# Piletskii-Oleg/chunkfs

Hardware: AMD Instinct MI355X
Metric: GiB/s chunked device-resident, FastCDC 4/8/16 KiB avg, at 1/2/4/8 MI355X (higher is better)
Workload: dtype u8

## Files before the change

chunkfs_amd/csrc/fastcdc.hip:

```cpp
#include "fastcdc.hpp"

#include <cstdlib>
#include <type_traits>

namespace cdc {
namespace p3 {
namespace {


constexpr uint32_t kCandPosMask = 0x00FFFFFFu;
constexpr uint32_t kCandHitL = 1u << 30;
constexpr uint32_t kCandHitS = 1u << 31;

typedef unsigned int u32x4 __attribute__((ext_vector_type(4)));
typedef const __attribute__((address_space(1))) u32x4 g_u32x4;
typedef const __attribute__((address_space(1))) uint8_t g_u8;
typedef const __attribute__((address_space(1))) uint32_t g_u32;
typedef __attribute__((address_space(1))) uint64_t g_u64;
__device__ __forceinline__ g_u32x4 *as_global4(const void *p) { return (g_u32x4 *)(p); }
__device__ __forceinline__ g_u8 *as_global1(const void *p) { return (g_u8 *)(p); }
__device__ __forceinline__ uint4 ld16(g_u32x4 *p) {
    const u32x4 v = *p;
    return make_uint4(v.x, v.y, v.z, v.w);
}
__device__ __forceinline__ uint4 ld16_nt(g_u32x4 *p) {
    const u32x4 v = __builtin_nontemporal_load(p);
    return make_uint4(v.x, v.y, v.z, v.w);
}

#ifndef CDC_SCAN_NOFENCE
#define SCHED_FENCE() __builtin_amdgcn_sched_barrier(0)
#else
#define SCHED_FENCE() do {} while (0)
#endif
#ifndef CDC_SCAN_WAVES
#define CDC_SCAN_WAVES 12
#endif
#ifndef CDC_SCAN_NT_ODD
#define CDC_SCAN_NT_ODD 1
#endif
#ifndef CDC_SCAN_WAVE_MAJOR
#define CDC_SCAN_WAVE_MAJOR 1
#endif
#ifndef CDC_SCAN_LOOK
#define CDC_SCAN_LOOK 1
#endif
#ifndef CDC_SCAN_TRUNC
#define CDC_SCAN_TRUNC 0
#endif

__device__ __forceinline__ void wave_sync_lds() {
    __builtin_amdgcn_fence(__ATOMIC_RELEASE, "wavefront");
    __builtin_amdgcn_wave_barrier();
    __builtin_amdgcn_fence(__ATOMIC_ACQUIRE, "wavefront");
}

__device__ __forceinline__ void locate(const StreamTable &st, uint64_t g, uint32_t &si, uint64_t &off) {
    uint32_t lo = 0, hi = st.n;
    while (hi - lo > 1) {
        const uint32_t mid = (lo + hi) >> 1;
        if (st.span_base[mid] <= g) lo = mid; else hi = mid;
    }
    si = lo;
    off = (g - st.span_base[lo]) << st.span_log2;
}

template <bool kAlign>
__device__ __forceinline__ uint32_t cand_test(uint64_t h, const FastParams &fp) {
    if constexpr (kAlign) {
        return (uint32_t)(h >> 32) & fp.cm32;
    } else {
        return ((uint32_t)h & fp.cm_lo) | ((uint32_t)(h >> 32) & fp.cm_hi);
    }
}

__device__ __forceinline__ uint64_t shl1_add(uint64_t h, uint64_t g) {
    return (h << 1) + g;
}

__device__ __forceinline__ uint64_t wave_shr1(uint64_t v, uint64_t fill) {
    const uint32_t lo = (uint32_t)__builtin_amdgcn_update_dpp(
        (int)(uint32_t)fill, (int)(uint32_t)v, 0x138, 0xF, 0xF, false);
    const uint32_t hi = (uint32_t)__builtin_amdgcn_update_dpp(
        (int)(uint32_t)(fill >> 32), (int)(uint32_t)(v >> 32), 0x138, 0xF, 0xF, false);
    return ((uint64_t)hi << 32) | lo;
}

__device__ __forceinline__ uint64_t readlane_u64(uint64_t v, int l) {
    const uint32_t lo = (uint32_t)__builtin_amdgcn_readlane((int)(uint32_t)v, l);
    const uint32_t hi = (uint32_t)__builtin_amdgcn_readlane((int)(uint32_t)(v >> 32), l);
    return ((uint64_t)hi << 32) | lo;
}

__device__ __forceinline__ uint64_t gear_prefix(uint64_t g, uint32_t lane) {
#pragma unroll
    for (int k = 1; k < 64; k <<= 1) {
        const uint64_t t = __shfl_up(g, k);
        if (lane >= (uint32_t)k) g += t << k;
    }
    return g;
}

constexpr uint32_t kTruncMax = 47;
constexpr uint32_t kTruncNone = 63;
constexpr uint32_t kTruncUnknown = 62;
constexpr int kRecTShift = 24;

struct Regime {
    uint64_t rem, a0, ce, re, tl;
};

__device__ __forceinline__ Regime regime(const FastParams &fp, uint64_t s, uint64_t n) {
    Regime R;
    uint64_t rem = n - s, center = fp.avg;
    if (rem > fp.max) rem = fp.max; else if (rem < center) center = rem;
    R.rem = rem;
    R.a0 = (fp.min / 2) * 2;
    R.ce = (center / 2) * 2;
    R.re = (rem / 2) * 2;
    R.tl = min(R.a0 + (uint64_t)fp.trunc, R.re);
    return R;
}


constexpr int kCopies = 32;
constexpr uint32_t kEntCap = 64;
constexpr uint32_t kStep = 64;

__device__ __forceinline__ uint64_t gear_of(const uint64_t *tab, uint32_t rep_off, uint32_t w, int b) {
    const uint32_t addr = __builtin_amdgcn_perm(rep_off, w, 0x0c0c0004u | ((uint32_t)b << 8));
    return *reinterpret_cast<const uint64_t *>(reinterpret_cast<const char *>(tab) + addr);
}

struct G4 {
    uint64_t v[4];
};

__device__ __forceinline__ void look4(G4 &g, const uint64_t *tab, uint32_t rep, uint32_t w) {
#pragma unroll
    for (int b = 0; b < 4; ++b) g.v[b] = gear_of(tab, rep, w, b);
}

template <bool kAlign>
__device__ __forceinline__ void chain4_test(uint64_t &h, uint32_t &acc, const G4 &g, const FastParams &fp) {
#pragma unroll
    for (int i = 0; i < 4; ++i) {
        h = shl1_add(h, g.v[i]);
        acc = min(acc, cand_test<kAlign>(h, fp));
    }
}

__device__ __forceinline__ uint32_t word_of(const uint4 &v, int w) {
    return w == 0 ? v.x : w == 1 ? v.y : w == 2 ? v.z : v.w;
}

__device__ __forceinline__ uint4 ld16_guarded(const uint8_t *base, uint32_t p, uint32_t limit) {
    if (p + 16 <= limit) return ld16(as_global4(base + p));
    uint32_t w[4] = {0, 0, 0, 0};
    if (p < limit) {
        g_u8 *gb = as_global1(base);
        for (uint32_t j = 0; p + j < limit; ++j) w[j >> 2] |= (uint32_t)gb[p + j] << (8 * j);
    }
    return make_uint4(w[0], w[1], w[2], w[3]);
}

struct EntryList {
    uint32_t *pos, *hlo, *hhi, *cnt;
};

constexpr uint32_t kEntFix = 1u << 31;
constexpr uint32_t kEntPos = kEntFix - 1;

__device__ __forceinline__ void append_hits(bool hit, uint32_t pos, uint64_t h0, uint32_t &ne,
                                            const EntryList &E) {
    const uint64_t m = __ballot(hit);
    if (m) {
        if (hit) {
            const uint32_t below = __builtin_amdgcn_mbcnt_hi((uint32_t)(m >> 32),
                                                             __builtin_amdgcn_mbcnt_lo((uint32_t)m, 0u));
            const uint32_t slot = ne + below;
            if (slot < kEntCap) {
                E.pos[slot] = pos;
                E.hlo[slot] = (uint32_t)h0;
                E.hhi[slot] = (uint32_t)(h0 >> 32);
            }
        }
        ne += (uint32_t)__popcll(m);
    }
}

__device__ __forceinline__ void append_hits_d(bool hit, uint32_t pos, uint64_t h0, const uint4 &q, uint32_t &ne,
                                              const EntryList &E, uint4 *edat) {
    const uint64_t m = __ballot(hit);
    if (m) {
        if (hit) {
            const uint32_t below = __builtin_amdgcn_mbcnt_hi((uint32_t)(m >> 32),
                                                             __builtin_amdgcn_mbcnt_lo((uint32_t)m, 0u));
            const uint32_t slot = ne + below;
            if (slot < kEntCap) {
                E.pos[slot] = pos;
                E.hlo[slot] = (uint32_t)h0;
                E.hhi[slot] = (uint32_t)(h0 >> 32);
                edat[slot] = q;
            }
        }
        ne += (uint32_t)__popcll(m);
    }
}

template <bool kAlign>
__device__ __forceinline__ uint32_t quarter(uint64_t &h, const uint4 &v, const uint64_t *tab, uint32_t rep,
                                            const FastParams &fp) {
    G4 ga, gb;
    uint32_t acc = 0xffffffffu;
    look4(ga, tab, rep, v.x);
    SCHED_FENCE();
    look4(gb, tab, rep, v.y);
    SCHED_FENCE();
    chain4_test<kAlign>(h, acc, ga, fp);
    SCHED_FENCE();
    look4(ga, tab, rep, v.z);
    SCHED_FENCE();
    chain4_test<kAlign>(h, acc, gb, fp);
    SCHED_FENCE();
    look4(gb, tab, rep, v.w);
    SCHED_FENCE();
    chain4_test<kAlign>(h, acc, ga, fp);
    SCHED_FENCE();
    chain4_test<kAlign>(h, acc, gb, fp);
    SCHED_FENCE();
    return acc;
}

struct Q4 {
    uint4 q[4];
};

template <bool kAlign, int kLook>
__device__ __forceinline__ void process_step(const Q4 &C, uint64_t &h, uint32_t pos0, uint32_t &ne,
                                             const EntryList &E, const uint64_t *tab, uint32_t rep,
                                             const FastParams &fp) {
    if constexpr (kLook == 1) {
        G4 ga, gb;
        look4(ga, tab, rep, C.q[0].x);
        SCHED_FENCE();
#pragma unroll
        for (int q = 0; q < 4; ++q) {
            const uint64_t h0 = h;
            uint32_t acc = 0xffffffffu;
#pragma unroll
            for (int w = 0; w < 4; w += 2) {
                look4(gb, tab, rep, word_of(C.q[q], w + 1));
                SCHED_FENCE();
                chain4_test<kAlign>(h, acc, ga, fp);
                SCHED_FENCE();
                if (q < 3 || w < 2) {
                    look4(ga, tab, rep, w < 2 ? word_of(C.q[q], w + 2) : word_of(C.q[q + 1], 0));
                    SCHED_FENCE();
                }
                chain4_test<kAlign>(h, acc, gb, fp);
                SCHED_FENCE();
            }
            append_hits(acc == 0, pos0 + 16 * q, h0, ne, E);
        }
    } else {
        G4 ga0, ga1, gb0, gb1;
        look4(ga0, tab, rep, C.q[0].x);
        look4(ga1, tab, rep, C.q[0].y);
        SCHED_FENCE();
#pragma unroll
        for (int q = 0; q < 4; ++q) {
            const uint64_t h0 = h;
            uint32_t acc = 0xffffffffu;
            look4(gb0, tab, rep, C.q[q].z);
            look4(gb1, tab, rep, C.q[q].w);
            SCHED_FENCE();
            chain4_test<kAlign>(h, acc, ga0, fp);
            chain4_test<kAlign>(h, acc, ga1, fp);
            SCHED_FENCE();
            if (q < 3) {
                look4(ga0, tab, rep, C.q[q + 1].x);
                look4(ga1, tab, rep, C.q[q + 1].y);
                SCHED_FENCE();
            }
            chain4_test<kAlign>(h, acc, gb0, fp);
            chain4_test<kAlign>(h, acc, gb1, fp);
            SCHED_FENCE();
            append_hits(acc == 0, pos0 + 16 * q, h0, ne, E);
        }
    }
}

template <bool kAlign>
__device__ __forceinline__ void process_step_d(const Q4 &C, uint64_t &h, uint32_t pos0, uint32_t &ne,
                                               const EntryList &E, uint4 *edat, const uint64_t *tab, uint32_t rep,
                                               const FastParams &fp) {
    G4 ga, gb;
    look4(ga, tab, rep, C.q[0].x);
    SCHED_FENCE();
#pragma unroll
    for (int q = 0; q < 4; ++q) {
        const uint64_t h0 = h;
        uint32_t acc = 0xffffffffu;
#pragma unroll
        for (int w = 0; w < 4; w += 2) {
            look4(gb, tab, rep, word_of(C.q[q], w + 1));
            SCHED_FENCE();
            chain4_test<kAlign>(h, acc, ga, fp);
            SCHED_FENCE();
            if (q < 3 || w < 2) {
                look4(ga, tab, rep, w < 2 ? word_of(C.q[q], w + 2) : word_of(C.q[q + 1], 0));
                SCHED_FENCE();
            }
            chain4_test<kAlign>(h, acc, gb, fp);
            SCHED_FENCE();
        }
        append_hits_d(acc == 0, pos0 + 16 * q, h0, C.q[q], ne, E, edat);
    }
}

template <bool kNt = false>
__device__ __forceinline__ void gload_step(Q4 &X, const uint8_t *gp, uint64_t istride, uint32_t t) {
#pragma unroll
    for (int i = 0; i < 4; ++i)
        X.q[i] = kNt ? ld16_nt(as_global4(gp + i * istride + t * kStep)) : ld16(as_global4(gp + i * istride + t * kStep));
}

__device__ __forceinline__ void stage_step(Q4 &C, const Q4 &X, uint4 *wrow, const uint4 *rrow) {
#pragma unroll
    for (int i = 0; i < 4; ++i) wrow[i * 16 * 5] = X.q[i];
    __builtin_amdgcn_wave_barrier();
#pragma unroll
    for (int k = 0; k < 4; ++k) C.q[k] = rrow[k];
    __builtin_amdgcn_wave_barrier();
}

typedef const __attribute__((address_space(3))) uint64_t lds_u64;
typedef const __attribute__((address_space(3))) char lds_char;

#if CDC_SCAN_TRUNC
__device__ __noinline__ uint32_t scan_trunc(const uint8_t *base, uint32_t c, uint64_t avail, lds_u64 *ltab,
                                            uint32_t rep, uint32_t mn, uint32_t avg, uint32_t mx, uint32_t trunc,
                                            uint64_t mask_s, uint64_t mask_l) {
    const uint32_t a0 = (mn / 2) * 2, ce = (avg / 2) * 2, re = (mx / 2) * 2;
    if (avail - c < (uint64_t)mx || (uint64_t)a0 + 52 > avail - c) return kTruncUnknown;
    const uint32_t tl = min(a0 + trunc, re);
    if (tl <= a0) return kTruncNone;
    const uint32_t len = tl - a0;
    const uint64_t w0 = (uint64_t)c + a0;
    const uint64_t al = w0 & ~3ull;
    const uint32_t sh = (uint32_t)(w0 - al);
    uint32_t w[13];
#pragma unroll
    for (int i = 0; i < 13; ++i) w[i] = *(g_u32 *)(base + al + 4 * i);
    uint64_t h = 0;
    uint32_t t = kTruncNone;
#pragma unroll
    for (int k = 0; k < 12; ++k) {
        const uint32_t a = __builtin_amdgcn_alignbyte(w[k + 1], w[k], sh);
#pragma unroll
        for (int j = 0; j < 4; ++j) {
            const uint32_t d = 4 * k + j;
            if (d >= kTruncMax) break;
            const uint32_t addr = __builtin_amdgcn_perm(rep, a, 0x0c0c0004u | ((uint32_t)j << 8));
            h = shl1_add(h, *reinterpret_cast<lds_u64 *>(reinterpret_cast<lds_char *>(ltab) + addr));
            const bool hit = d < len && !(h & ((a0 + d) < ce ? mask_s : mask_l));
            t = (hit && t == kTruncNone) ? d : t;
        }
    }
    return t;
}

#endif

__device__ __forceinline__ void flush_span(uint64_t g, const uint8_t *base, uint32_t span_len, uint64_t avail,
                                           uint32_t sub_mask, uint32_t ne, const EntryList &E, const uint64_t *tab,
                                           uint32_t rep, const FastParams &fp, const Candidates &cand,
                                           uint32_t lane, const uint4 *edat = nullptr) {
    wave_sync_lds();
    uint32_t *cpos = cand.pos + g * cand.cap;
    if (ne > kEntCap) {
        if (lane == 0) cand.count[g] = cand.cap + 1;
        wave_sync_lds();
        return;
    }
    uint32_t hs = 0, hl = 0, my_pos = 0;
    const uint32_t wd = lane < ne ? E.pos[lane] : 0u;
    const bool keep = lane < ne && ((wd & kEntFix) || (wd & sub_mask) >= 48);
    if (lane < ne) E.cnt[lane] = 0;
    if (keep) {
        my_pos = wd & kEntPos;
        uint64_t hh = ((uint64_t)E.hhi[lane] << 32) | E.hlo[lane];
        const uint4 v = edat ? edat[lane] : ld16_guarded(base, my_pos, span_len);
#pragma unroll
        for (int w = 0; w < 4; ++w)
#pragma unroll
            for (int b = 0; b < 4; ++b) {
                const int j = 4 * w + b;
                hh = (hh << 1) + gear_of(tab, rep, word_of(v, w), b);
                if (my_pos + j < span_len) {
                    hs |= (uint32_t)((hh & fp.mask_s_sh) == 0) << j;
                    hl |= (uint32_t)((hh & fp.mask_l_sh) == 0) << j;
                }
            }
        E.cnt[lane] = __popc(hs | hl);
    }
    wave_sync_lds();
    uint32_t slot = 0, total = 0;
    for (uint32_t k = 0; k < ne; ++k) {
        const uint32_t c = E.cnt[k];
        total += c;
        if ((E.pos[k] & kEntPos) < my_pos) slot += c;
    }
    if (keep) {
        for (uint32_t m = hs | hl; m; m &= m - 1) {
            const uint32_t j = __builtin_ctz(m);
            uint32_t t = kTruncUnknown;
#if CDC_SCAN_TRUNC
            t = scan_trunc(base, my_pos + j, avail, (lds_u64 *)tab, rep, fp.min, fp.avg, fp.max, fp.trunc,
                           fp.mask_s_sh, fp.mask_l_sh);
#endif
            if (slot < cand.cap)
                cpos[slot] = (my_pos + j) | (t << kRecTShift) | (((hs >> j) & 1u) << 31) | (((hl >> j) & 1u) << 30);
            ++slot;
        }
    }
    if (lane == 0) cand.count[g] = total;
    wave_sync_lds();
}

template <int kW>
struct ScanLds {
    uint64_t tab[256 * kCopies];
    uint4 stage[kW][64 * 5];
    uint32_t epos[kW][kEntCap];
    uint32_t ehlo[kW][kEntCap];
    uint32_t ehhi[kW][kEntCap];
    uint32_t ecnt[kW][kEntCap];
};

template <bool kAlign, int kW, int kLook, int kMode>
__global__ __launch_bounds__(kW * 64, 1) void scan_kernel(const StreamTable st, const FastParams fp,
                                                           const uint64_t *__restrict__ gear,
                                                           const Candidates cand, const Compact cp) {
    __shared__ ScanLds<kW> L;
    const uint64_t *tab = L.tab;
    for (int i = threadIdx.x; i < 256 * kCopies; i += kW * 64)
        L.tab[i] = gear[i / kCopies] << fp.tshift;
    if (blockIdx.x == 0 && threadIdx.x < kStatWords) cp.stats[threadIdx.x] = 0;
    __syncthreads();

    const uint32_t lane = threadIdx.x & 63;
    const uint32_t wave = threadIdx.x >> 6;
    const uint32_t rep = (lane & 31) * 8;
    const uint64_t span = 1ull << st.span_log2;
    const uint32_t sub_log2 = st.span_log2 - 6;
    const uint32_t sub = 1u << sub_log2;
    const uint32_t steps = sub / kStep;
    const uint32_t lo = lane << sub_log2;
    const uint64_t istride = 16ull * sub;
    const EntryList E{L.epos[wave], L.ehlo[wave], L.ehhi[wave], L.ecnt[wave]};
    const uint32_t rsel = ((lane >> 3) & 3) + 8 * (lane >> 5) + 4 * ((lane >> 2) & 1);
    uint4 *wrow = &L.stage[wave][rsel * 5 + (lane & 3)];
    const uint4 *rrow = &L.stage[wave][lane * 5];

    const uint64_t gstride = (uint64_t)gridDim.x * kW;
    auto next_full = [&](uint64_t g, uint32_t &si, uint64_t &off) {
        for (; g < st.total_spans; g += gstride) {
            locate(st, g, si, off);
            if (st.lens[si] - off >= span) break;
        }
        return g;
    };
    Q4 A, B, C;
    uint32_t si, wb = 0;
    uint64_t off;
    uint64_t g = next_full(CDC_SCAN_WAVE_MAJOR ? (uint64_t)wave * gridDim.x + blockIdx.x
                                               : (uint64_t)blockIdx.x * kW + wave, si, off);
    const uint8_t *base = nullptr, *gp = nullptr;
    auto prefetch = [&]() {
        base = st.ptrs[si] + off;
        gp = base + (uint64_t)rsel * sub + (lane & 3) * 16;
        wb = 0;
        if (off != 0 && lane < 48) wb = as_global1(base)[(int)lane - 48];
        gload_step(A, gp, istride, 0);
        SCHED_FENCE();
        gload_step<(bool)CDC_SCAN_NT_ODD>(B, gp, istride, 1);
        SCHED_FENCE();
    };
    if (g < st.total_spans) prefetch();
    while (g < st.total_spans) {
        uint32_t ne = 0;
        uint64_t h = 0;
        uint4 F0, F1, F2;
        stage_step(C, A, wrow, rrow);
        F0 = C.q[0];
        F1 = C.q[1];
        F2 = C.q[2];
        gload_step(A, gp, istride, 2);
        SCHED_FENCE();
#define CDC_PROC(POS)                                                                          \
    do {                                                                                       \
        if constexpr (kMode == 1) h ^= (uint64_t)(C.q[0].x ^ C.q[1].y ^ C.q[2].z ^ C.q[3].w);   \
        else process_step<kAlign, kLook>(C, h, POS, ne, E, tab, rep, fp);                      \
    } while (0)
#define CDC_SCAN_PAIR(T, LOAD_B, STAGE_A, LOAD_A)                                              \
    do {                                                                                       \
        CDC_PROC(lo + (T) * kStep);                                                            \
        SCHED_FENCE();                                                                         \
        stage_step(C, B, wrow, rrow);                                                          \
        if (LOAD_B && kMode != 2) gload_step<(bool)CDC_SCAN_NT_ODD>(B, gp, istride, (T) + 3);  \
        SCHED_FENCE();                                                                         \
        CDC_PROC(lo + ((T) + 1) * kStep);                                                      \
        SCHED_FENCE();                                                                         \
        if (STAGE_A) stage_step(C, A, wrow, rrow);                                             \
        if (LOAD_A && kMode != 2) gload_step(A, gp, istride, (T) + 4);                         \
        SCHED_FENCE();                                                                         \
    } while (0)
        uint32_t t = 0;
        for (; t + 4 < steps; t += 2) CDC_SCAN_PAIR(t, true, true, true);
        CDC_SCAN_PAIR(t, true, true, false);
        CDC_SCAN_PAIR(t + 2, false, false, false);
#undef CDC_SCAN_PAIR
#undef CDC_PROC
        const uint64_t g_cur = g, off_cur = off;
        const uint64_t avail_cur = st.lens[si] - off;
        const uint32_t wb_cur = wb;
        const uint8_t *base_cur = base;
        g = next_full(g + gstride, si, off);
        if (g < st.total_spans) prefetch();
        const uint64_t gw = lane < 48 ? L.tab[wb_cur * kCopies + (lane & 31)] : 0;
        const uint64_t hw = readlane_u64(gear_prefix(gw, lane), 47);
        h = wave_shr1(h, off_cur != 0 ? hw : 0);
        {
            uint64_t h0 = h;
            append_hits(quarter<kAlign>(h, F0, tab, rep, fp) == 0, lo | kEntFix, h0, ne, E);
            h0 = h;
            append_hits(quarter<kAlign>(h, F1, tab, rep, fp) == 0, (lo + 16) | kEntFix, h0, ne, E);
            h0 = h;
            append_hits(quarter<kAlign>(h, F2, tab, rep, fp) == 0, (lo + 32) | kEntFix, h0, ne, E);
        }
        flush_span(g_cur, base_cur, (uint32_t)span, avail_cur, sub - 1, ne, E, tab, rep, fp, cand, lane);
    }
    if (fp.diag & 64) {
        __syncthreads();
        if (threadIdx.x == 0)
            atomicMax((unsigned long long *)&cp.stats[kStatDiag0 + 6],
                      (unsigned long long)__builtin_amdgcn_s_memrealtime());
    }
}


constexpr int kDmaW = 8;
constexpr uint32_t kDiagDmaScan = 1024;

struct ScanDmaLds {
    uint64_t tab[256 * kCopies];
    uint4 ring[kDmaW][2][256];
    uint32_t epos[kDmaW][kEntCap];
    uint32_t ehlo[kDmaW][kEntCap];
    uint32_t ehhi[kDmaW][kEntCap];
    uint32_t ecnt[kDmaW][kEntCap];
    uint4 edat[kDmaW][kEntCap];
    uint32_t carry[kDmaW][64];
    uint4 recs[kDmaW][64];
};

typedef const __attribute__((address_space(4))) uint64_t c_u64;
typedef const __attribute__((address_space(4))) uint32_t c_u32;

__device__ __forceinline__ uint64_t cld(const uint64_t *p) { return *(c_u64 *)p; }

__device__ __forceinline__ void glds16(const uint8_t *gsrc, uint32_t lds_dst) {
    uint32_t keep;
    asm volatile("s_mov_b32 %0, m0\n\ts_mov_b32 m0, %2\n\ts_nop 0\n\tglobal_load_lds_dwordx4 %1, off\n\ts_mov_b32 m0, %0"
                 : "=&s"(keep)
                 : "v"(gsrc), "s"(lds_dst)
                 : "memory");
}

template <int N>
__device__ __forceinline__ void wait_vm() {
    asm volatile("s_waitcnt vmcnt(%0)" ::"i"(N) : "memory");
}

__device__ __forceinline__ void glds4(const uint8_t *gsrc, uint32_t lds_dst) {
    uint32_t keep;
    asm volatile("s_mov_b32 %0, m0\n\ts_mov_b32 m0, %2\n\ts_nop 0\n\tglobal_load_lds_dword %1, off\n\ts_mov_b32 m0, %0"
                 : "=&s"(keep)
                 : "v"(gsrc), "s"(lds_dst)
                 : "memory");
}

template <int kCtrl, int kRowMask>
__device__ __forceinline__ uint64_t dpp64(uint64_t v) {
    const uint32_t lo = (uint32_t)__builtin_amdgcn_update_dpp(0, (int)(uint32_t)v, kCtrl, kRowMask, 0xF, false);
    const uint32_t hi = (uint32_t)__builtin_amdgcn_update_dpp(0, (int)(uint32_t)(v >> 32), kCtrl, kRowMask, 0xF, false);
    return ((uint64_t)hi << 32) | lo;
}

__device__ __forceinline__ uint64_t wave_total_dpp(uint64_t v) {
    v += dpp64<0x111, 0xF>(v);
    v += dpp64<0x112, 0xF>(v);
    v += dpp64<0x114, 0xF>(v);
    v += dpp64<0x118, 0xF>(v);
    v += dpp64<0x142, 0xA>(v);
    v += dpp64<0x143, 0xC>(v);
    return readlane_u64(v, 63);
}

__device__ __forceinline__ void flush_span_d(uint64_t g, uint32_t sub_mask, uint32_t ne, const EntryList &E,
                                             const uint4 *edat, uint4 *recs, const uint64_t *tab, uint32_t rep,
                                             const FastParams &fp, const Candidates &cand, uint32_t lane) {
    wave_sync_lds();
    uint32_t hs = 0, hl = 0, my_pos = 0xFFFFFFFFu, cnt = 0;
    const bool ovf = ne > kEntCap;
    const uint32_t wd = lane < ne && !ovf ? E.pos[lane] : 0u;
    const bool keep = lane < ne && !ovf && ((wd & kEntFix) || (wd & sub_mask) >= 48);
    if (keep) {
        my_pos = wd & kEntPos;
        uint64_t hh = ((uint64_t)E.hhi[lane] << 32) | E.hlo[lane];
        const uint4 v = edat[lane];
#pragma unroll
        for (int w = 0; w < 4; ++w)
#pragma unroll
            for (int b = 0; b < 4; ++b) {
                const int j = 4 * w + b;
                hh = (hh << 1) + gear_of(tab, rep, word_of(v, w), b);
                hs |= (uint32_t)((hh & fp.mask_s_sh) == 0) << j;
                hl |= (uint32_t)((hh & fp.mask_l_sh) == 0) << j;
            }
        cnt = __popc(hs | hl);
    }
    uint32_t slot = 0, total = 0;
    const uint32_t nk = ovf ? 0u : ne;
    for (uint32_t k = 0; k < nk; ++k) {
        const uint32_t pk = (uint32_t)__builtin_amdgcn_readlane((int)my_pos, (int)k);
        const uint32_t ck = (uint32_t)__builtin_amdgcn_readlane((int)cnt, (int)k);
        total += ck;
        slot += pk < my_pos ? ck : 0u;
    }
    uint32_t *const rec = reinterpret_cast<uint32_t *>(recs);
    if (keep) {
        for (uint32_t m = hs | hl; m; m &= m - 1) {
            const uint32_t j = __builtin_ctz(m);
            if (slot < cand.cap)
                rec[slot] = (my_pos + j) | (kTruncUnknown << kRecTShift) | (((hs >> j) & 1u) << 31) |
                            (((hl >> j) & 1u) << 30);
            ++slot;
        }
    }
    wave_sync_lds();
    if (lane < cand.cap / 4)
        *reinterpret_cast<uint4 *>(cand.pos + g * cand.cap + 4 * lane) = recs[lane];
    if (lane == 0) cand.count[g] = ovf ? cand.cap + 1 : total;
    wave_sync_lds();
}

__device__ __forceinline__ void locate_c(const StreamTable &st, uint64_t g, uint32_t &si, uint64_t &off) {
    uint32_t lo = 0, hi = st.n;
    while (hi - lo > 1) {
        const uint32_t mid = (lo + hi) >> 1;
        if (cld(st.span_base + mid) <= g) lo = mid; else hi = mid;
    }
    si = lo;
    off = (g - cld(st.span_base + lo)) << st.span_log2;
}

template <bool kAlign>
__global__ __launch_bounds__(kDmaW * 64, 1) void scan_dma_kernel(const StreamTable st, const FastParams fp,
                                                                 const uint64_t *__restrict__ gear,
                                                                 const Candidates cand, const Compact cp) {
    __shared__ ScanDmaLds L;
    const uint64_t *tab = L.tab;
    for (int i = threadIdx.x; i < 256 * kCopies; i += kDmaW * 64)
        L.tab[i] = gear[i / kCopies] << fp.tshift;
    if (blockIdx.x == 0 && threadIdx.x < kStatWords) cp.stats[threadIdx.x] = 0;
    __syncthreads();

    const uint32_t lane = threadIdx.x & 63;
    const uint32_t wave = __builtin_amdgcn_readfirstlane(threadIdx.x >> 6);
    const uint32_t rep = (lane & 31) * 8;
    const uint64_t span = 1ull << st.span_log2;
    const uint32_t sub_log2 = st.span_log2 - 6;
    const uint32_t sub = 1u << sub_log2;
    const uint32_t steps = sub / kStep;
    const uint32_t lo = lane << sub_log2;
    const EntryList E{L.epos[wave], L.ehlo[wave], L.ehhi[wave], L.ecnt[wave]};
    uint4 *const edat = L.edat[wave];
    const uint64_t src_lane = (uint64_t)(lane & 15) * sub + (lane >> 4) * 16;
    const uint64_t istride = 16ull * sub;
    const uint32_t ring0 = (uint32_t)(uintptr_t)&L.ring[wave][0][0];
    const uint4 *rd0 = &L.ring[wave][0][(lane >> 4) * 64 + (lane & 15)];
    const uint64_t gstride = (uint64_t)gridDim.x * kDmaW;
    auto next_full = [&](uint64_t g, uint32_t &si, uint64_t &off) {
        for (; g < st.total_spans; g += gstride) {
            locate_c(st, g, si, off);
            if (cld(st.lens + si) - off >= span) break;
        }
        return g;
    };
    auto stream_ptr = [&](uint32_t si) {
        return reinterpret_cast<const uint8_t *>(cld(reinterpret_cast<const uint64_t *>(st.ptrs) + si));
    };
    auto issue = [&](const uint8_t *src, uint32_t slot) {
#pragma unroll
        for (int i = 0; i < 4; ++i) glds16(src + i * istride, ring0 + slot * 4096 + i * 1024);
    };
    const uint32_t carry0 = (uint32_t)(uintptr_t)&L.carry[wave][0];
    auto issue_carry = [&](const uint8_t *b, uint64_t o) {
        glds4(o != 0 ? b - 48 + 4 * (lane % 12) : b, carry0);
    };
    uint32_t si;
    uint64_t off;
    uint64_t g = next_full(CDC_SCAN_WAVE_MAJOR ? (uint64_t)wave * gridDim.x + blockIdx.x
                                               : (uint64_t)blockIdx.x * kDmaW + wave, si, off);
    const uint8_t *base = nullptr;
    if (g < st.total_spans) {
        base = stream_ptr(si) + off;
        issue_carry(base, off);
        issue(base + src_lane, 0);
        issue(base + src_lane + kStep, 1);
    }
    uint32_t slot = 0;
    bool first = true;
    while (g < st.total_spans) {
        const uint64_t g_cur = g, off_cur = off;
        const uint8_t *const base_cur = base;
        g = next_full(g + gstride, si, off);
        const bool more = g < st.total_spans;
        const uint8_t *const base_next = more ? stream_ptr(si) + off : base_cur;
        const uint64_t off_next = more ? off : 0;
        uint32_t ne = 0;
        uint64_t h = 0;
        uint32_t wb = 0;
        uint4 F0, F1, F2;
        for (uint32_t t = 0; t < steps; ++t) {
            if (t == 0) {
                if (first) wait_vm<4>(); else wait_vm<6>();
            } else if (t + 1 == steps) {
                wait_vm<5>();
            } else {
                wait_vm<4>();
            }
            Q4 C;
            const uint4 *rd = rd0 + slot * 256;
#pragma unroll
            for (int k = 0; k < 4; ++k) C.q[k] = rd[k * 16];
            if (t == 0 && lane < 48) wb = L.carry[wave][lane >> 2];
            asm volatile("s_waitcnt lgkmcnt(0)" ::: "memory");
            if (t + 2 < steps) {
                issue(base_cur + src_lane + (t + 2) * kStep, slot);
            } else if (t + 2 == steps) {
                issue_carry(base_next, off_next);
                issue(base_next + src_lane, slot);
            } else {
                issue(base_next + src_lane + kStep, slot);
            }
            if (t == 0) {
                F0 = C.q[0];
                F1 = C.q[1];
                F2 = C.q[2];
            }
            process_step_d<kAlign>(C, h, lo + t * kStep, ne, E, edat, tab, rep, fp);
            slot ^= 1;
        }
        first = false;
        base = base_next;
        wb = (wb >> (8 * (lane & 3))) & 0xFFu;
        const uint64_t gw = lane < 48 ? L.tab[wb * kCopies + (lane & 31)] << (47 - lane) : 0;
        const uint64_t hw = wave_total_dpp(gw);
        h = wave_shr1(h, off_cur != 0 ? hw : 0);
        {
            uint64_t h0 = h;
            append_hits_d(quarter<kAlign>(h, F0, tab, rep, fp) == 0, lo | kEntFix, h0, F0, ne, E, edat);
            h0 = h;
            append_hits_d(quarter<kAlign>(h, F1, tab, rep, fp) == 0, (lo + 16) | kEntFix, h0, F1, ne, E, edat);
            h0 = h;
            append_hits_d(quarter<kAlign>(h, F2, tab, rep, fp) == 0, (lo + 32) | kEntFix, h0, F2, ne, E, edat);
        }
        flush_span_d(g_cur, sub - 1, ne, E, edat, L.recs[wave], tab, rep, fp, cand, lane);
    }
    wait_vm<0>();
}

template <bool kAlign>
__global__ __launch_bounds__(64) void scan_tail_kernel(const StreamTable st, const FastParams fp,
                                                       const uint64_t *__restrict__ gear, const Candidates cand,
                                                       const uint64_t *__restrict__ tails) {
    __shared__ uint64_t tab[256 * kCopies];
    __shared__ uint32_t e_pos[kEntCap], e_hlo[kEntCap], e_hhi[kEntCap], e_cnt[kEntCap];
    for (int i = threadIdx.x; i < 256 * kCopies; i += 64) tab[i] = gear[i / kCopies] << fp.tshift;
    __syncthreads();
    const uint32_t lane = threadIdx.x;
    const uint32_t rep = (lane & 31) * 8;
    const uint64_t g = tails[blockIdx.x];
    const EntryList E{e_pos, e_hlo, e_hhi, e_cnt};
    uint32_t si;
    uint64_t off;
    locate(st, g, si, off);
    const uint8_t *base = st.ptrs[si] + off;
    const uint32_t span_len = (uint32_t)(st.lens[si] - off);
    const uint32_t sub_log2 = st.span_log2 - 6;
    const uint32_t sub = 1u << sub_log2;
    const uint32_t lo = lane << sub_log2;
    uint32_t ne = 0;
    uint64_t h = 0;
    const bool active = lo < span_len;
    if (active && off + lo != 0) {
        (void)quarter<kAlign>(h, ld16(as_global4(base + lo - 48)), tab, rep, fp);
        (void)quarter<kAlign>(h, ld16(as_global4(base + lo - 32)), tab, rep, fp);
        (void)quarter<kAlign>(h, ld16(as_global4(base + lo - 16)), tab, rep, fp);
    }
    for (uint32_t it = 0; it < sub / 16; ++it) {
        const uint32_t p = lo + 16 * it;
        bool hit = false;
        const uint64_t h0 = h;
        if (active && p < span_len) hit = quarter<kAlign>(h, ld16_guarded(base, p, span_len), tab, rep, fp) == 0;
        append_hits(hit, p | kEntFix, h0, ne, E);
    }
    flush_span(g, base, span_len, span_len, 0, ne, E, tab, rep, fp, cand, lane);
}



#ifndef CDC_RES_WAVES
#define CDC_RES_WAVES 8
#endif
#ifndef CDC_WALK_SPANS
#define CDC_WALK_SPANS 8
#endif
#ifndef CDC_WIN_RECS
#define CDC_WIN_RECS 768
#endif
constexpr int kResWaves = CDC_RES_WAVES;
#ifndef CDC_RES_LINK_DIAG
#define CDC_RES_LINK_DIAG 0
#endif
#ifndef CDC_RES_HOSTREL
#define CDC_RES_HOSTREL 1
#endif
#ifndef CDC_WALK_COOP
#define CDC_WALK_COOP 1
#endif
#ifndef CDC_RES_FASTTRUNC
#define CDC_RES_FASTTRUNC 1
#endif
constexpr int kResThreads = kResWaves * 64;

__device__ __forceinline__ uint32_t trunc_words(const uint8_t *data, uint64_t w0, uint32_t len, uint64_t a0,
                                                uint64_t ce, uint64_t mask_s, uint64_t mask_l, lds_u64 *tab) {
    const uint64_t al = w0 & ~3ull;
    const uint32_t sh = (uint32_t)(w0 - al);
    uint32_t w[13];
#pragma unroll
    for (int i = 0; i < 13; ++i) w[i] = *(g_u32 *)(data + al + 4 * i);
    uint64_t h = 0;
    uint32_t t = kTruncNone;
#pragma unroll
    for (int k = 0; k < 12; ++k) {
        const uint32_t a = __builtin_amdgcn_alignbyte(w[k + 1], w[k], sh);
#pragma unroll
        for (int j = 0; j < 4; ++j) {
            const uint32_t d = 4 * k + j;
            if (d >= kTruncMax) break;
            h = shl1_add(h, tab[(a >> (8 * j)) & 255]);
            const bool hit = d < len && !(h & ((a0 + d) < ce ? mask_s : mask_l));
            t = (hit && t == kTruncNone) ? d : t;
        }
    }
    return t;
}

#ifndef CDC_RES_CALLS
#define CDC_RES_CALLS __forceinline__
#endif
__device__ CDC_RES_CALLS uint32_t trunc_at(const uint8_t *data, uint64_t n, uint64_t c, uint64_t mask_s,
                                          uint64_t mask_l, uint32_t mn, uint32_t avg, uint32_t mx, uint32_t trunc,
                                          lds_u64 *tab) {
    if (n - c <= mn) return kTruncNone;
    uint64_t rem = n - c, center = avg;
    if (rem > mx) rem = mx; else if (rem < center) center = rem;
    const uint64_t a0 = (mn / 2) * 2, ce = (center / 2) * 2, re = (rem / 2) * 2;
    const uint64_t tl = min(a0 + (uint64_t)trunc, re);
    if (tl <= a0) return kTruncNone;
    const uint32_t len = (uint32_t)(tl - a0);
    const uint64_t w0 = c + a0;
    if ((w0 & ~3ull) + 52 <= n) return trunc_words(data, w0, len, a0, ce, mask_s, mask_l, tab);
    uint64_t h = 0;
    for (uint32_t d = 0; d < len; ++d) {
        h = (h << 1) + tab[as_global1(data)[w0 + d]];
        if (!(h & ((a0 + d) < ce ? mask_s : mask_l))) return d;
    }
    return kTruncNone;
}

__device__ __forceinline__ uint32_t trunc_call(const uint8_t *data, uint64_t n, uint64_t c, const FastParams &fp,
                                               const uint64_t *tab) {
    return trunc_at(data, n, c, fp.mask_s, fp.mask_l, fp.min, fp.avg, fp.max, fp.trunc, (lds_u64 *)tab);
}

__device__ CDC_RES_CALLS uint64_t coop_next_bytes(uint32_t mn, uint32_t avg, uint32_t mx, uint64_t mask_s,
                                                 uint64_t mask_l, const uint64_t *tab, const uint8_t *data,
                                                 uint64_t n, uint64_t s, uint32_t lane) {
    if (n - s <= mn) return n;
    FastParams fp{};
    fp.min = mn;
    fp.avg = avg;
    fp.max = mx;
    const Regime R = regime(fp, s, n);
    uint64_t h = 0;
    for (uint64_t b = R.a0; b < R.re; b += 64) {
        const uint64_t p1 = min(b + 64, R.re);
        const uint64_t p = b + lane;
        const bool in = p < p1;
        const uint64_t gv = in ? tab[as_global1(data)[s + p]] : 0;
        const uint64_t x = gear_prefix(gv, lane) + ((h << lane) << 1);
        const bool hit = in && !(x & (p < R.ce ? mask_s : mask_l));
        const uint64_t m = __ballot(hit);
        if (m) return s + b + (uint64_t)(__ffsll((long long)m) - 1);
        h = __shfl(x, (int)(p1 - b - 1));
    }
    return s + R.rem;
}

__device__ __forceinline__ void load_tab1(uint64_t *tab, const uint64_t *gear) {
    for (int i = threadIdx.x; i < 256; i += blockDim.x) tab[i] = gear[i];
    __syncthreads();
}

__device__ __forceinline__ uint64_t wave_sum(uint64_t v) {
#pragma unroll
    for (int k = 1; k < 64; k <<= 1) v += __shfl_xor(v, k);
    return v;
}

__device__ __forceinline__ uint64_t lane_next_global(const StreamTable &st, const FastParams &fp,
                                                     const Candidates &cand, const uint64_t *tab,
                                                     const uint8_t *data, uint64_t n, uint64_t gbase, uint64_t s) {
    if (n - s <= fp.min) return n;
    const Regime R = regime(fp, s, n);
    const uint32_t t = trunc_call(data, n, s, fp, tab);
    if (t != kTruncNone) return s + R.a0 + t;
    if (R.tl >= R.re) return s + R.rem;
    const uint64_t lo = s + R.tl, hi = s + R.re;
    for (uint64_t sp = lo >> st.span_log2; (sp << st.span_log2) < hi; ++sp) {
        const uint64_t g = gbase + sp;
        const uint32_t cnt = cand.count[g];
        if (cnt > cand.cap) return ~0ull;
        const uint32_t *P = cand.pos + g * cand.cap;
        const uint64_t sp0 = sp << st.span_log2;
        const uint32_t lo_rel = lo > sp0 ? (uint32_t)(lo - sp0) : 0u;
        uint32_t a = 0, b = cnt;
        while (a < b) {
            const uint32_t m = (a + b) >> 1;
            if ((P[m] & kCandPosMask) < lo_rel) a = m + 1; else b = m;
        }
        for (uint32_t j = a; j < cnt; ++j) {
            const uint32_t r = P[j];
            const uint64_t c = sp0 + (r & kCandPosMask);
            if (c >= hi) return s + R.rem;
            if (r & ((c - s) < R.ce ? kCandHitS : kCandHitL)) return c;
        }
    }
    return s + R.rem;
}

struct LaneSpan {
    bool act, first;
    uint32_t si;
    uint64_t g, off, span_end, n, gbase;
    const uint8_t *data;
};

// ... 901 lines not shown
```

Measured before the change: 4244.

## Pack hit entries into AoS LDS records and cache stream span lookup

Replaces the separate per-field LDS arrays (pos/hlo/hhi/cnt plus optional edat) with a packed Entry struct holding a 16-byte key and the 16-byte data, so every scan path stores the data words and flush never re-reads global memory. Adds a branch-light exact_flags using v_min/lshl_or for the aligned case, a vectorized gear-table fill, and a StreamCursor that skips the binary search when consecutive spans fall in the same stream. This costs more LDS per wave and more LDS writes per hit in the non-DMA scan path.

After: 4271, median of 6. Within noise of the previous version (+0.6%).

```diff
diff --git a/chunkfs_amd/csrc/fastcdc.hip b/chunkfs_amd/csrc/fastcdc.hip
--- a/chunkfs_amd/csrc/fastcdc.hip
+++ b/chunkfs_amd/csrc/fastcdc.hip
@@ -164,47 +164,26 @@
     return make_uint4(w[0], w[1], w[2], w[3]);
 }
 
-struct EntryList {
-    uint32_t *pos, *hlo, *hhi, *cnt;
+struct Entry {
+    uint4 key;
+    uint4 dat;
 };
 
 constexpr uint32_t kEntFix = 1u << 31;
 constexpr uint32_t kEntPos = kEntFix - 1;
 
-__device__ __forceinline__ void append_hits(bool hit, uint32_t pos, uint64_t h0, uint32_t &ne,
-                                            const EntryList &E) {
+__device__ __forceinline__ void append_hits(bool hit, uint32_t pos, uint64_t h0, const uint4 &q, uint32_t &ne,
+                                            Entry *E) {
     const uint64_t m = __ballot(hit);
     if (m) {
-        if (hit) {
-            const uint32_t below = __builtin_amdgcn_mbcnt_hi((uint32_t)(m >> 32),
-                                                             __builtin_amdgcn_mbcnt_lo((uint32_t)m, 0u));
-            const uint32_t slot = ne + below;
-            if (slot < kEntCap) {
-                E.pos[slot] = pos;
-                E.hlo[slot] = (uint32_t)h0;
-                E.hhi[slot] = (uint32_t)(h0 >> 32);
-            }
-        }
-        ne += (uint32_t)__popcll(m);
-    }
-}
-
-__device__ __forceinline__ void append_hits_d(bool hit, uint32_t pos, uint64_t h0, const uint4 &q, uint32_t &ne,
-                                              const EntryList &E, uint4 *edat) {
-    const uint64_t m = __ballot(hit);
-    if (m) {
-        if (hit) {
-            const uint32_t below = __builtin_amdgcn_mbcnt_hi((uint32_t)(m >> 32),
-                                                             __builtin_amdgcn_mbcnt_lo((uint32_t)m, 0u));
-            const uint32_t slot = ne + below;
-            if (slot < kEntCap) {
-                E.pos[slot] = pos;
-                E.hlo[slot] = (uint32_t)h0;
-                E.hhi[slot] = (uint32_t)(h0 >> 32);
-                edat[slot] = q;
-            }
-        }
-        ne += (uint32_t)__popcll(m);
+        const uint32_t n1 = ne + (uint32_t)__popcll(m);
+        if (hit && n1 <= kEntCap) {
+            const uint32_t slot = __builtin_amdgcn_mbcnt_hi((uint32_t)(m >> 32),
+                                                            __builtin_amdgcn_mbcnt_lo((uint32_t)m, ne));
+            E[slot].key = make_uint4(pos, 0u, (uint32_t)h0, (uint32_t)(h0 >> 32));
+            E[slot].dat = q;
+        }
+        ne = n1;
     }
 }
 
@@ -238,7 +217,7 @@
 
 template <bool kAlign, int kLook>
 __device__ __forceinline__ void process_step(const Q4 &C, uint64_t &h, uint32_t pos0, uint32_t &ne,
-                                             const EntryList &E, const uint64_t *tab, uint32_t rep,
+                                             Entry *E, const uint64_t *tab, uint32_t rep,
                                              const FastParams &fp) {
     if constexpr (kLook == 1) {
         G4 ga, gb;
@@ -261,7 +240,7 @@
                 chain4_test<kAlign>(h, acc, gb, fp);
                 SCHED_FENCE();
             }
-            append_hits(acc == 0, pos0 + 16 * q, h0, ne, E);
+            append_hits(acc == 0, pos0 + 16 * q, h0, C.q[q], ne, E);
         }
     } else {
         G4 ga0, ga1, gb0, gb1;
@@ -286,36 +265,8 @@
             chain4_test<kAlign>(h, acc, gb0, fp);
             chain4_test<kAlign>(h, acc, gb1, fp);
             SCHED_FENCE();
-            append_hits(acc == 0, pos0 + 16 * q, h0, ne, E);
-        }
-    }
-}
-
-template <bool kAlign>
-__device__ __forceinline__ void process_step_d(const Q4 &C, uint64_t &h, uint32_t pos0, uint32_t &ne,
-                                               const EntryList &E, uint4 *edat, const uint64_t *tab, uint32_t rep,
-                                               const FastParams &fp) {
-    G4 ga, gb;
-    look4(ga, tab, rep, C.q[0].x);
-    SCHED_FENCE();
-#pragma unroll
-    for (int q = 0; q < 4; ++q) {
-        const uint64_t h0 = h;
-        uint32_t acc = 0xffffffffu;
-#pragma unroll
-        for (int w = 0; w < 4; w += 2) {
-            look4(gb, tab, rep, word_of(C.q[q], w + 1));
-            SCHED_FENCE();
-            chain4_test<kAlign>(h, acc, ga, fp);
-            SCHED_FENCE();
-            if (q < 3 || w < 2) {
-                look4(ga, tab, rep, w < 2 ? word_of(C.q[q], w + 2) : word_of(C.q[q + 1], 0));
-                SCHED_FENCE();
-            }
-            chain4_test<kAlign>(h, acc, gb, fp);
-            SCHED_FENCE();
-        }
-        append_hits_d(acc == 0, pos0 + 16 * q, h0, C.q[q], ne, E, edat);
+            append_hits(acc == 0, pos0 + 16 * q, h0, C.q[q], ne, E);
+        }
     }
 }
 
@@ -373,10 +324,49 @@
 
 #endif
 
+__device__ __forceinline__ uint32_t shift_in_nz(uint32_t acc, uint32_t x) {
+    uint32_t r;
+    asm("v_min_u32 %0, 1, %2\n\tv_lshl_or_b32 %0, %1, 1, %0" : "=&v"(r) : "v"(acc), "v"(x));
+    return r;
+}
+
+template <bool kAlign>
+__device__ __forceinline__ void exact_flags(uint64_t hh, const uint4 &v, const uint64_t *tab, uint32_t rep,
+                                            const FastParams &fp, uint32_t &hs, uint32_t &hl) {
+    if constexpr (kAlign) {
+        uint32_t ms = (uint32_t)(fp.mask_s_sh >> 32), ml = (uint32_t)(fp.mask_l_sh >> 32);
+        asm("" : "+s"(ms), "+s"(ml));
+        uint32_t ns = 0, nl = 0;
+#pragma unroll
+        for (int w = 0; w < 4; ++w)
+#pragma unroll
+            for (int b = 0; b < 4; ++b) {
+                hh = (hh << 1) + gear_of(tab, rep, word_of(v, w), b);
+                const uint32_t hi = (uint32_t)(hh >> 32);
+                ns = shift_in_nz(ns, hi & ms);
+                nl = shift_in_nz(nl, hi & ml);
+            }
+        hs = ~__brev(ns) >> 16;
+        hl = ~__brev(nl) >> 16;
+    } else {
+        hs = hl = 0;
+#pragma unroll
+        for (int w = 0; w < 4; ++w)
+#pragma unroll
+            for (int b = 0; b < 4; ++b) {
+                const int j = 4 * w + b;
+                hh = (hh << 1) + gear_of(tab, rep, word_of(v, w), b);
+                hs |= (uint32_t)((hh & fp.mask_s_sh) == 0) << j;
+                hl |= (uint32_t)((hh & fp.mask_l_sh) == 0) << j;
+            }
+    }
+}
+
+template <bool kAlign, bool kFull>
 __device__ __forceinline__ void flush_span(uint64_t g, const uint8_t *base, uint32_t span_len, uint64_t avail,
-                                           uint32_t sub_mask, uint32_t ne, const EntryList &E, const uint64_t *tab,
+                                           uint32_t sub_mask, uint32_t ne, Entry *E, const uint64_t *tab,
                                            uint32_t rep, const FastParams &fp, const Candidates &cand,
-                                           uint32_t lane, const uint4 *edat = nullptr) {
+                                           uint32_t lane) {
     wave_sync_lds();
     uint32_t *cpos = cand.pos + g * cand.cap;
     if (ne > kEntCap) {
@@ -385,32 +375,26 @@
         return;
     }
     uint32_t hs = 0, hl = 0, my_pos = 0;
-    const uint32_t wd = lane < ne ? E.pos[lane] : 0u;
+    const uint4 key = lane < ne ? E[lane].key : make_uint4(0u, 0u, 0u, 0u);
+    const uint32_t wd = key.x;
     const bool keep = lane < ne && ((wd & kEntFix) || (wd & sub_mask) >= 48);
-    if (lane < ne) E.cnt[lane] = 0;
     if (keep) {
         my_pos = wd & kEntPos;
-        uint64_t hh = ((uint64_t)E.hhi[lane] << 32) | E.hlo[lane];
-        const uint4 v = edat ? edat[lane] : ld16_guarded(base, my_pos, span_len);
-#pragma unroll
-        for (int w = 0; w < 4; ++w)
-#pragma unroll
-            for (int b = 0; b < 4; ++b) {
-                const int j = 4 * w + b;
-                hh = (hh << 1) + gear_of(tab, rep, word_of(v, w), b);
-                if (my_pos + j < span_len) {
-                    hs |= (uint32_t)((hh & fp.mask_s_sh) == 0) << j;
-                    hl |= (uint32_t)((hh & fp.mask_l_sh) == 0) << j;
-                }
-            }
-        E.cnt[lane] = __popc(hs | hl);
+        exact_flags<kAlign>(((uint64_t)key.w << 32) | key.z, E[lane].dat, tab, rep, fp, hs, hl);
+        if constexpr (!kFull) {
+            const uint32_t left = span_len - my_pos;
+            const uint32_t valid = left < 16 ? (1u << left) - 1 : 0xFFFFu;
+            hs &= valid;
+            hl &= valid;
+        }
+        E[lane].key.y = __popc(hs | hl);
     }
     wave_sync_lds();
     uint32_t slot = 0, total = 0;
     for (uint32_t k = 0; k < ne; ++k) {
-        const uint32_t c = E.cnt[k];
-        total += c;
-        if ((E.pos[k] & kEntPos) < my_pos) slot += c;
+        const uint2 pc = *reinterpret_cast<const uint2 *>(&E[k].key);
+        total += pc.y;
+        if ((pc.x & kEntPos) < my_pos) slot += pc.y;
     }
     if (keep) {
         for (uint32_t m = hs | hl; m; m &= m - 1) {
@@ -429,14 +413,63 @@
     wave_sync_lds();
 }
 
+template <int kThreads>
+__device__ __forceinline__ void fill_gear_tab(uint64_t *tab, const uint64_t *__restrict__ gear, uint32_t tshift) {
+    constexpr int kPer = kThreads / 16;
+    constexpr int kRounds = (256 + kPer - 1) / kPer;
+    constexpr int kBatch = kRounds < 8 ? kRounds : 8;
+    static_assert(kThreads % 16 == 0 && kRounds % kBatch == 0, "fill_gear_tab: block shape");
+    uint4 *tab4 = reinterpret_cast<uint4 *>(tab);
+    const uint32_t c = threadIdx.x & 15, e0 = threadIdx.x >> 4;
+    for (int r0 = 0; r0 < kRounds; r0 += kBatch) {
+        uint64_t v[kBatch];
+#pragma unroll
+        for (int r = 0; r < kBatch; ++r) {
+            const uint32_t e = e0 + (uint32_t)(r0 + r) * kPer;
+            v[r] = e < 256 ? gear[e] : 0;
+        }
+#pragma unroll
+        for (int r = 0; r < kBatch; ++r) {
+            const uint32_t e = e0 + (uint32_t)(r0 + r) * kPer;
+            const uint64_t x = v[r] << tshift;
+            if (e < 256) tab4[e * (kCopies / 2) + c] = make_uint4((uint32_t)x, (uint32_t)(x >> 32), (uint32_t)x, (uint32_t)(x >> 32));
+        }
+    }
+}
+
+typedef const __attribute__((address_space(4))) uint64_t c_u64;
+
+__device__ __forceinline__ uint64_t cld(const uint64_t *p) { return *(c_u64 *)p; }
+
+struct StreamCursor {
+    uint64_t first = 0, next = 0, len = 0;
+    const uint8_t *ptr = nullptr;
+};
+
+__device__ __forceinline__ uint64_t next_full_span(const StreamTable &st, StreamCursor &sc, uint64_t g,
+                                                   uint64_t gstride) {
+    for (; g < st.total_spans; g += gstride) {
+        if (g >= sc.next) {
+            uint32_t lo = 0, hi = st.n;
+            while (hi - lo > 1) {
+                const uint32_t mid = (lo + hi) >> 1;
+                if (cld(st.span_base + mid) <= g) lo = mid; else hi = mid;
+            }
+            sc.first = cld(st.span_base + lo);
+            sc.next = cld(st.span_base + lo + 1);
+            sc.len = cld(st.lens + lo);
+            sc.ptr = reinterpret_cast<const uint8_t *>(cld(reinterpret_cast<const uint64_t *>(st.ptrs) + lo));
+        }
+        if (g - sc.first < (sc.len >> st.span_log2)) break;
+    }
+    return g;
+}
+
 template <int kW>
 struct ScanLds {
     uint64_t tab[256 * kCopies];
     uint4 stage[kW][64 * 5];
-    uint32_t epos[kW][kEntCap];
-    uint32_t ehlo[kW][kEntCap];
-    uint32_t ehhi[kW][kEntCap];
-    uint32_t ecnt[kW][kEntCap];
+    Entry ent[kW][kEntCap];
 };
 
 template <bool kAlign, int kW, int kLook, int kMode>
@@ -445,13 +478,12 @@
                                                            const Candidates cand, const Compact cp) {
     __shared__ ScanLds<kW> L;
     const uint64_t *tab = L.tab;
-    for (int i = threadIdx.x; i < 256 * kCopies; i += kW * 64)
-        L.tab[i] = gear[i / kCopies] << fp.tshift;
+    fill_gear_tab<kW * 64>(L.tab, gear, fp.tshift);
     if (blockIdx.x == 0 && threadIdx.x < kStatWords) cp.stats[threadIdx.x] = 0;
     __syncthreads();
 
     const uint32_t lane = threadIdx.x & 63;
-    const uint32_t wave = threadIdx.x >> 6;
+    const uint32_t wave = __builtin_amdgcn_readfirstlane(threadIdx.x >> 6);
     const uint32_t rep = (lane & 31) * 8;
     const uint64_t span = 1ull << st.span_log2;
     const uint32_t sub_log2 = st.span_log2 - 6;
@@ -459,27 +491,22 @@
     const uint32_t steps = sub / kStep;
     const uint32_t lo = lane << sub_log2;
     const uint64_t istride = 16ull * sub;
-    const EntryList E{L.epos[wave], L.ehlo[wave], L.ehhi[wave], L.ecnt[wave]};
+    Entry *const E = L.ent[wave];
     const uint32_t rsel = ((lane >> 3) & 3) + 8 * (lane >> 5) + 4 * ((lane >> 2) & 1);
     uint4 *wrow = &L.stage[wave][rsel * 5 + (lane & 3)];
     const uint4 *rrow = &L.stage[wave][lane * 5];
 
     const uint64_t gstride = (uint64_t)gridDim.x * kW;
-    auto next_full = [&](uint64_t g, uint32_t &si, uint64_t &off) {
-        for (; g < st.total_spans; g += gstride) {
-            locate(st, g, si, off);
-            if (st.lens[si] - off >= span) break;
-        }
-        return g;
-    };
+    StreamCursor sc;
     Q4 A, B, C;
-    uint32_t si, wb = 0;
-    uint64_t off;
-    uint64_t g = next_full(CDC_SCAN_WAVE_MAJOR ? (uint64_t)wave * gridDim.x + blockIdx.x
-                                               : (uint64_t)blockIdx.x * kW + wave, si, off);
+    uint32_t wb = 0;
+    uint64_t off = 0;
+    uint64_t g = next_full_span(st, sc, CDC_SCAN_WAVE_MAJOR ? (uint64_t)wave * gridDim.x + blockIdx.x
+                                                            : (uint64_t)blockIdx.x * kW + wave, gstride);
     const uint8_t *base = nullptr, *gp = nullptr;
     auto prefetch = [&]() {
-        base = st.ptrs[si] + off;
+        off = (g - sc.first) << st.span_log2;
+        base = sc.ptr + off;
         gp = base + (uint64_t)rsel * sub + (lane & 3) * 16;
         wb = 0;
         if (off != 0 && lane < 48) wb = as_global1(base)[(int)lane - 48];
@@ -524,23 +551,24 @@
 #undef CDC_SCAN_PAIR
 #undef CDC_PROC
         const uint64_t g_cur = g, off_cur = off;
-        const uint64_t avail_cur = st.lens[si] - off;
+        const uint64_t avail_cur = sc.len - off;
         const uint32_t wb_cur = wb;
         const uint8_t *base_cur = base;
-        g = next_full(g + gstride, si, off);
+        g = next_full_span(st, sc, g + gstride, gstride);
         if (g < st.total_spans) prefetch();
         const uint64_t gw = lane < 48 ? L.tab[wb_cur * kCopies + (lane & 31)] : 0;
         const uint64_t hw = readlane_u64(gear_prefix(gw, lane), 47);
         h = wave_shr1(h, off_cur != 0 ? hw : 0);
         {
             uint64_t h0 = h;
-            append_hits(quarter<kAlign>(h, F0, tab, rep, fp) == 0, lo | kEntFix, h0, ne, E);
+            append_hits(quarter<kAlign>(h, F0, tab, rep, fp) == 0, lo | kEntFix, h0, F0, ne, E);
             h0 = h;
-            append_hits(quarter<kAlign>(h, F1, tab, rep, fp) == 0, (lo + 16) | kEntFix, h0, ne, E);
+            append_hits(quarter<kAlign>(h, F1, tab, rep, fp) == 0, (lo + 16) | kEntFix, h0, F1, ne, E);
             h0 = h;
-            append_hits(quarter<kAlign>(h, F2, tab, rep, fp) == 0, (lo + 32) | kEntFix, h0, ne, E);
-        }
-        flush_span(g_cur, base_cur, (uint32_t)span, avail_cur, sub - 1, ne, E, tab, rep, fp, cand, lane);
+            append_hits(quarter<kAlign>(h, F2, tab, rep, fp) == 0, (lo + 32) | kEntFix, h0, F2, ne, E);
+        }
+        flush_span<kAlign, true>(g_cur, base_cur, (uint32_t)span, avail_cur, sub - 1, ne, E, tab, rep, fp, cand,
+                                 lane);
     }
     if (fp.diag & 64) {
         __syncthreads();
@@ -557,19 +585,10 @@
 struct ScanDmaLds {
     uint64_t tab[256 * kCopies];
     uint4 ring[kDmaW][2][256];
-    uint32_t epos[kDmaW][kEntCap];
-    uint32_t ehlo[kDmaW][kEntCap];
-    uint32_t ehhi[kDmaW][kEntCap];
-    uint32_t ecnt[kDmaW][kEntCap];
-    uint4 edat[kDmaW][kEntCap];
+    Entry ent[kDmaW][kEntCap];
     uint32_t carry[kDmaW][64];
     uint4 recs[kDmaW][64];
 };
-
-typedef const __attribute__((address_space(4))) uint64_t c_u64;
-typedef const __attribute__((address_space(4))) uint32_t c_u32;
-
-__device__ __forceinline__ uint64_t cld(const uint64_t *p) { return *(c_u64 *)p; }
 
 __device__ __forceinline__ void glds16(const uint8_t *gsrc, uint32_t lds_dst) {
     uint32_t keep;
@@ -609,27 +628,19 @@
     return readlane_u64(v, 63);
 }
 
-__device__ __forceinline__ void flush_span_d(uint64_t g, uint32_t sub_mask, uint32_t ne, const EntryList &E,
-                                             const uint4 *edat, uint4 *recs, const uint64_t *tab, uint32_t rep,
+template <bool kAlign>
+__device__ __forceinline__ void flush_span_d(uint64_t g, uint32_t sub_mask, uint32_t ne, const Entry *E,
+                                             uint4 *recs, const uint64_t *tab, uint32_t rep,
                                              const FastParams &fp, const Candidates &cand, uint32_t lane) {
     wave_sync_lds();
     uint32_t hs = 0, hl = 0, my_pos = 0xFFFFFFFFu, cnt = 0;
     const bool ovf = ne > kEntCap;
-    const uint32_t wd = lane < ne && !ovf ? E.pos[lane] : 0u;
+    const uint4 key = lane < ne && !ovf ? E[lane].key : make_uint4(0u, 0u, 0u, 0u);
+    const uint32_t wd = key.x;
     const bool keep = lane < ne && !ovf && ((wd & kEntFix) || (wd & sub_mask) >= 48);
     if (keep) {
         my_pos = wd & kEntPos;
-        uint64_t hh = ((uint64_t)E.hhi[lane] << 32) | E.hlo[lane];
-        const uint4 v = edat[lane];
-#pragma unroll
-        for (int w = 0; w < 4; ++w)
-#pragma unroll
-            for (int b = 0; b < 4; ++b) {
-                const int j = 4 * w + b;
-                hh = (hh << 1) + gear_of(tab, rep, word_of(v, w), b);
-                hs |= (uint32_t)((hh & fp.mask_s_sh) == 0) << j;
-                hl |= (uint32_t)((hh & fp.mask_l_sh) == 0) << j;
-            }
+        exact_flags<kAlign>(((uint64_t)key.w << 32) | key.z, E[lane].dat, tab, rep, fp, hs, hl);
         cnt = __popc(hs | hl);
     }
     uint32_t slot = 0, total = 0;
@@ -657,52 +668,30 @@
     wave_sync_lds();
 }
 
-__device__ __forceinline__ void locate_c(const StreamTable &st, uint64_t g, uint32_t &si, uint64_t &off) {
-    uint32_t lo = 0, hi = st.n;
-    while (hi - lo > 1) {
-        const uint32_t mid = (lo + hi) >> 1;
-        if (cld(st.span_base + mid) <= g) lo = mid; else hi = mid;
-    }
-    si = lo;
-    off = (g - cld(st.span_base + lo)) << st.span_log2;
-}
-
 template <bool kAlign>
 __global__ __launch_bounds__(kDmaW * 64, 1) void scan_dma_kernel(const StreamTable st, const FastParams fp,
                                                                  const uint64_t *__restrict__ gear,
                                                                  const Candidates cand, const Compact cp) {
     __shared__ ScanDmaLds L;
     const uint64_t *tab = L.tab;
-    for (int i = threadIdx.x; i < 256 * kCopies; i += kDmaW * 64)
-        L.tab[i] = gear[i / kCopies] << fp.tshift;
+    fill_gear_tab<kDmaW * 64>(L.tab, gear, fp.tshift);
     if (blockIdx.x == 0 && threadIdx.x < kStatWords) cp.stats[threadIdx.x] = 0;
     __syncthreads();
 
     const uint32_t lane = threadIdx.x & 63;
     const uint32_t wave = __builtin_amdgcn_readfirstlane(threadIdx.x >> 6);
     const uint32_t rep = (lane & 31) * 8;
-    const uint64_t span = 1ull << st.span_log2;
     const uint32_t sub_log2 = st.span_log2 - 6;
     const uint32_t sub = 1u << sub_log2;
     const uint32_t steps = sub / kStep;
     const uint32_t lo = lane << sub_log2;
-    const EntryList E{L.epos[wave], L.ehlo[wave], L.ehhi[wave], L.ecnt[wave]};
-    uint4 *const edat = L.edat[wave];
+    Entry *const E = L.ent[wave];
     const uint64_t src_lane = (uint64_t)(lane & 15) * sub + (lane >> 4) * 16;
     const uint64_t istride = 16ull * sub;
     const uint32_t ring0 = (uint32_t)(uintptr_t)&L.ring[wave][0][0];
     const uint4 *rd0 = &L.ring[wave][0][(lane >> 4) * 64 + (lane & 15)];
     const uint64_t gstride = (uint64_t)gridDim.x * kDmaW;
-    auto next_full = [&](uint64_t g, uint32_t &si, uint64_t &off) {
-        for (; g < st.total_spans; g += gstride) {
-            locate_c(st, g, si, off);
-            if (cld(st.lens + si) - off >= span) break;
-        }
-        return g;
-    };
-    auto stream_ptr = [&](uint32_t si) {
-        return reinterpret_cast<const uint8_t *>(cld(reinterpret_cast<const uint64_t *>(st.ptrs) + si));
-    };
+    StreamCursor sc;
     auto issue = [&](const uint8_t *src, uint32_t slot) {
 #pragma unroll
         for (int i = 0; i < 4; ++i) glds16(src + i * istride, ring0 + slot * 4096 + i * 1024);
@@ -711,13 +700,13 @@
     auto issue_carry = [&](const uint8_t *b, uint64_t o) {
         glds4(o != 0 ? b - 48 + 4 * (lane % 12) : b, carry0);
     };
-    uint32_t si;
-    uint64_t off;
-    uint64_t g = next_full(CDC_SCAN_WAVE_MAJOR ? (uint64_t)wave * gridDim.x + blockIdx.x
-                                               : (uint64_t)blockIdx.x * kDmaW + wave, si, off);
+    uint64_t off = 0;
+    uint64_t g = next_full_span(st, sc, CDC_SCAN_WAVE_MAJOR ? (uint64_t)wave * gridDim.x + blockIdx.x
+                                                            : (uint64_t)blockIdx.x * kDmaW + wave, gstride);
     const uint8_t *base = nullptr;
     if (g < st.total_spans) {
-        base = stream_ptr(si) + off;
+        off = (g - sc.first) << st.span_log2;
+        base = sc.ptr + off;
         issue_carry(base, off);
         issue(base + src_lane, 0);
         issue(base + src_lane + kStep, 1);
@@ -727,9 +716,10 @@
     while (g < st.total_spans) {
         const uint64_t g_cur = g, off_cur = off;
         const uint8_t *const base_cur = base;
-        g = next_full(g + gstride, si, off);
+        g = next_full_span(st, sc, g + gstride, gstride);
         const bool more = g < st.total_spans;
-        const uint8_t *const base_next = more ? stream_ptr(si) + off : base_cur;
+        if (more) off = (g - sc.first) << st.span_log2;
+        const uint8_t *const base_next = more ? sc.ptr + off : base_cur;
         const uint64_t off_next = more ? off : 0;
         uint32_t ne = 0;
         uint64_t h = 0;
@@ -762,7 +752,7 @@
                 F1 = C.q[1];
                 F2 = C.q[2];
             }
-            process_step_d<kAlign>(C, h, lo + t * kStep, ne, E, edat, tab, rep, fp);
+            process_step<kAlign, 1>(C, h, lo + t * kStep, ne, E, tab, rep, fp);
             slot ^= 1;
         }
         first = false;
@@ -773,13 +763,13 @@
         h = wave_shr1(h, off_cur != 0 ? hw : 0);
         {
             uint64_t h0 = h;
-            append_hits_d(quarter<kAlign>(h, F0, tab, rep, fp) == 0, lo | kEntFix, h0, F0, ne, E, edat);
+            append_hits(quarter<kAlign>(h, F0, tab, rep, fp) == 0, lo | kEntFix, h0, F0, ne, E);
             h0 = h;
-            append_hits_d(quarter<kAlign>(h, F1, tab, rep, fp) == 0, (lo + 16) | kEntFix, h0, F1, ne, E, edat);
+            append_hits(quarter<kAlign>(h, F1, tab, rep, fp) == 0, (lo + 16) | kEntFix, h0, F1, ne, E);
             h0 = h;
-            append_hits_d(quarter<kAlign>(h, F2, tab, rep, fp) == 0, (lo + 32) | kEntFix, h0, F2, ne, E, edat);
-        }
-        flush_span_d(g_cur, sub - 1, ne, E, edat, L.recs[wave], tab, rep, fp, cand, lane);
+            append_hits(quarter<kAlign>(h, F2, tab, rep, fp) == 0, (lo + 32) | kEntFix, h0, F2, ne, E);
+        }
+        flush_span_d<kAlign>(g_cur, sub - 1, ne, E, L.recs[wave], tab, rep, fp, cand, lane);
     }
     wait_vm<0>();
 }
@@ -789,13 +779,12 @@
                                                        const uint64_t *__restrict__ gear, const Candidates cand,
                                                        const uint64_t *__restrict__ tails) {
     __shared__ uint64_t tab[256 * kCopies];
-    __shared__ uint32_t e_pos[kEntCap], e_hlo[kEntCap], e_hhi[kEntCap], e_cnt[kEntCap];
-    for (int i = threadIdx.x; i < 256 * kCopies; i += 64) tab[i] = gear[i / kCopies] << fp.tshift;
+    __shared__ Entry E[kEntCap];
+    fill_gear_tab<64>(tab, gear, fp.tshift);
     __syncthreads();
     const uint32_t lane = threadIdx.x;
     const uint32_t rep = (lane & 31) * 8;
     const uint64_t g = tails[blockIdx.x];
-    const EntryList E{e_pos, e_hlo, e_hhi, e_cnt};
     uint32_t si;
     uint64_t off;
     locate(st, g, si, off);
@@ -816,10 +805,14 @@
         const uint32_t p = lo + 16 * it;
         bool hit = false;
         const uint64_t h0 = h;
-        if (active && p < span_len) hit = quarter<kAlign>(h, ld16_guarded(base, p, span_len), tab, rep, fp) == 0;
-        append_hits(hit, p | kEntFix, h0, ne, E);
-    }
-    flush_span(g, base, span_len, span_len, 0, ne, E, tab, rep, fp, cand, lane);
+        uint4 v = make_uint4(0u, 0u, 0u, 0u);
+        if (active && p < span_len) {
+            v = ld16_guarded(base, p, span_len);
+            hit = quarter<kAlign>(h, v, tab, rep, fp) == 0;
+        }
+        append_hits(hit, p | kEntFix, h0, v, ne, E);
+    }
+    flush_span<kAlign, false>(g, base, span_len, span_len, 0, ne, E, tab, rep, fp, cand, lane);
 }
 
 
```
